# alenzhao/Mitty

Hardware: NVIDIA B200
Metric: read pairs/sec (2x150, FASTQ-formatted, corrupted) (higher is better)
Workload: dtype u8

## Files before the change

### mitty_b200/csrc/mg_core.cuh

```cuda
#pragma once
#include <stdint.h>

#if defined(__CUDACC__)
#define MG_HD __host__ __device__ __forceinline__
#else
#define MG_HD inline
#endif
#if defined(__CUDACC__)
#define MG_NI static __host__ __device__ __noinline__ __attribute__((unused))
#else
#define MG_NI static __attribute__((noinline, unused))
#endif
#if defined(__CUDA_ARCH__)
#define MG_UNROLL _Pragma("unroll")
#define MG_NOUNROLL _Pragma("unroll 1")
#else
#define MG_UNROLL
#define MG_NOUNROLL
#endif


struct alignas(16) MgNode {
  uint32_t key;
  int32_t pr;
// ... 1 lines not shown
  uint32_t op;
};

#define MG_EXC_CASE 1u
struct alignas(16) MgExc {
  uint32_t start;
  uint32_t len;
  uint32_t byte;
  uint32_t pad;
};


MG_HD uint32_t mg_funnel_r(uint32_t lo, uint32_t hi, uint32_t sh) {
#if defined(__CUDA_ARCH__)
  return __funnelshift_r(lo, hi, sh);
#else
  return sh ? ((lo >> sh) | (hi << (32 - sh))) : lo;
#endif
}

MG_HD uint32_t mg_funnel_l(uint32_t lo, uint32_t hi, uint32_t sh) {
#if defined(__CUDA_ARCH__)
  return __funnelshift_l(lo, hi, sh);
#else
  return sh ? ((hi << sh) | (lo >> (32 - sh))) : hi;
#endif
}

MG_HD uint32_t mg_brev(uint32_t x) {
#if defined(__CUDA_ARCH__)
  return __brev(x);
#else
  x = ((x >> 1) & 0x55555555u) | ((x & 0x55555555u) << 1);
  x = ((x >> 2) & 0x33333333u) | ((x & 0x33333333u) << 2);
  x = ((x >> 4) & 0x0F0F0F0Fu) | ((x & 0x0F0F0F0Fu) << 4);
  x = ((x >> 8) & 0x00FF00FFu) | ((x & 0x00FF00FFu) << 8);
  return (x >> 16) | (x << 16);
#endif
}

MG_HD uint32_t mg_prmt(uint32_t a, uint32_t sel) {
#if defined(__CUDA_ARCH__)
  return __byte_perm(a, 0u, sel);
#else
  uint32_t r = 0;
  for (int i = 0; i < 4; i++) r |= ((a >> (8 * ((sel >> (4 * i)) & 3))) & 0xFFu) << (8 * i);
  return r;
#endif
}

MG_HD uint32_t mg_prmt2(uint32_t a, uint32_t b, uint32_t sel) {
#if defined(__CUDA_ARCH__)
  return __byte_perm(a, b, sel);
#else
  const uint64_t ab = ((uint64_t)b << 32) | a;
  uint32_t r = 0;
  for (int i = 0; i < 4; i++) r |= (uint32_t)((ab >> (8 * ((sel >> (4 * i)) & 7))) & 0xFFu) << (8 * i);
  return r;
#endif
}

template <class P>
MG_HD uint32_t mg_codes16(P seq, int64_t s) {
  int64_t w = s >> 4;
  uint32_t sh = (uint32_t)(s & 15) * 2u;
  uint32_t lo = seq[w];
  uint32_t hi = sh ? seq[w + 1] : 0u;
  return mg_funnel_r(lo, hi, sh);
}

MG_HD uint32_t mg_revcomp16(uint32_t x) {
  uint32_t y = mg_brev(x);
  y = ((y >> 1) & 0x55555555u) | ((y & 0x55555555u) << 1);
  return ~y;
}

MG_HD uint32_t mg_chars4(uint32_t b) {
  uint32_t y = (b | (b << 4)) & 0x0F0Fu;
  uint32_t z = (y | (y << 2)) & 0x3333u;
  return mg_prmt(0x54474341u , z);
}

MG_HD uint32_t mg_base_code(uint8_t c) {
  return c == 'A' ? 0u : c == 'C' ? 1u : c == 'G' ? 2u : c == 'T' ? 3u : 4u;
}


struct MgPhilox { uint32_t v[4]; };

MG_HD void mg_mulhilo(uint32_t a, uint32_t b, uint32_t &hi, uint32_t &lo) {
  uint64_t p = (uint64_t)a * (uint64_t)b;
  hi = (uint32_t)(p >> 32); lo = (uint32_t)p;
}

template <int ROUNDS>
MG_HD MgPhilox mg_philox_r(uint32_t c0, uint32_t c1, uint32_t c2, uint32_t c3, uint32_t k0, uint32_t k1) {
  MG_UNROLL
  for (int r = 0; r < ROUNDS; r++) {
    uint32_t h0, l0, h1, l1;
    mg_mulhilo(0xD2511F53u, c0, h0, l0);
    mg_mulhilo(0xCD9E8D57u, c2, h1, l1);
    uint32_t n0 = h1 ^ c1 ^ k0, n2 = h0 ^ c3 ^ k1;
    c0 = n0; c1 = l1; c2 = n2; c3 = l0;
    k0 += 0x9E3779B9u; k1 += 0xBB67AE85u;
  }
  MgPhilox o; o.v[0] = c0; o.v[1] = c1; o.v[2] = c2; o.v[3] = c3;
  return o;
}

MG_HD MgPhilox mg_philox(uint32_t c0, uint32_t c1, uint32_t c2, uint32_t c3, uint32_t k0, uint32_t k1) {
  return mg_philox_r<10>(c0, c1, c2, c3, k0, k1);
}

#define MG_CORRUPT_ROUNDS 7
MG_HD MgPhilox mg_philox_corrupt(uint32_t c0, uint32_t c1, uint32_t c2, uint32_t k0, uint32_t k1) {
  return mg_philox_r<MG_CORRUPT_ROUNDS>(c0, c1, c2, 0x636f7272u , k0, k1);
}

MG_HD double mg_u53(uint32_t a, uint32_t b) {
  return ((double)(a >> 5) * 67108864.0 + (double)(b >> 6)) / 9007199254740992.0;
}

#define MG_STREAM_GAP 0x67617073u
#define MG_STREAM_TLEN 0x746c656eu
#define MG_STREAM_CORRUPT 0x636f7272u

MG_HD uint32_t mg_feistel_round(uint32_t r, uint32_t k) {
  uint32_t x = r * 0x9E3779B1u + k;
  x ^= x >> 15; x *= 0x85EBCA77u; x ^= x >> 13; x *= 0xC2B2AE3Du; x ^= x >> 16;
  return x;
}

MG_HD uint32_t mg_perm_bits(uint32_t n) {
  uint32_t bits = 2;
  while (bits < 32 && (1ull << bits) < (unsigned long long)n) bits++;
  return bits;
}

MG_HD uint32_t mg_permute(uint32_t i, uint32_t n, uint32_t bits, uint32_t k0, uint32_t k1) {
  const uint32_t wa = bits >> 1, ma = (1u << wa) - 1u, mb = (bits - wa >= 32u) ? 0xFFFFFFFFu : (1u << (bits - wa)) - 1u;
  do {
    uint32_t a = i & ma, b = (i >> wa) & mb;
    MG_UNROLL
    for (int t = 0; t < 6; t += 2) {
      a ^= mg_feistel_round(b, k0 + (uint32_t)t) & ma;
      b ^= mg_feistel_round(a, k1 + (uint32_t)t + 1u) & mb;
    }
    i = (b << wa) | a;
  } while (i >= n);
  return i;
}


MG_HD uint32_t mg_pow10(int d) {
  switch (d) {
    case 0: return 1u; case 1: return 10u; case 2: return 100u; case 3: return 1000u; case 4: return 10000u;
    case 5: return 100000u; case 6: return 1000000u; case 7: return 10000000u; case 8: return 100000000u;
    default: return 1000000000u;
  }
}

MG_HD int mg_ndigits_ones(uint32_t v, uint32_t &ones) {
  int d = 1; uint32_t o = 1u;
  if (v >= 10u) { d++; o += 10u; }
  if (v >= 100u) { d++; o += 100u; }
  if (v >= 1000u) { d++; o += 1000u; }
  if (v >= 10000u) { d++; o += 10000u; }
  if (v >= 100000u) { d++; o += 100000u; }
  if (v >= 1000000u) { d++; o += 1000000u; }
  if (v >= 10000000u) { d++; o += 10000000u; }
  if (v >= 100000000u) { d++; o += 100000000u; }
  if (v >= 1000000000u) { d++; o += 1000000000u; }
  ones = o;
  return d;
}

MG_HD int mg_ndigits32(uint32_t v) { uint32_t o; return mg_ndigits_ones(v, o); }

MG_HD int mg_ndigits(uint64_t v) {
  if (v <= 0xFFFFFFFFull) return mg_ndigits32((uint32_t)v);
  int d = 1;
  while (v >= 10) { v /= 10; d++; }
  return d;
}


MG_HD uint64_t mg_digit_sum(uint64_t m) {
  if (m == 0) return 0;
  if (m <= 0xFFFFFFFFull) {
    uint32_t ones;
    const int d = mg_ndigits_ones((uint32_t)m, ones);
    return (uint64_t)d * (m + 1) - (uint64_t)ones;
  }
  const int d = mg_ndigits(m);
  uint64_t ones = 0, p = 1;
  for (int k = 0; k < d; k++) { ones += p; p *= 10; }
  return (uint64_t)d * (m + 1) - ones;
}


struct MgCountWriter {
  static constexpr bool is_bytes = false;
  uint32_t n;
  MG_HD void put(uint8_t) { n++; }
  MG_HD void put_word(uint32_t) { n += 4; }
};

struct MgGenericSpace {
  static constexpr bool is_generic = true;
  typedef uint8_t *ptr;
  static MG_HD void st8(ptr p, uint8_t v) { *p = v; }
  static MG_HD void st32(ptr p, uint32_t v) { *reinterpret_cast<uint32_t *>(p) = v; }
  static MG_HD uint32_t ld32(ptr p) { return *reinterpret_cast<const uint32_t *>(p); }
  static MG_HD uint32_t ld8(ptr p) { return *p; }
  static MG_HD uint32_t low2(ptr p) { return (uint32_t)((uintptr_t)p & 3); }
};
#if defined(__CUDACC__)
struct MgSharedSpace {
  static constexpr bool is_generic = false;
  typedef uint32_t ptr;
  static __device__ __forceinline__ void st8(ptr p, uint8_t v) { asm volatile("st.shared.u8 [%0], %1;" ::"r"(p), "r"((uint32_t)v)); }
  static __device__ __forceinline__ void st32(ptr p, uint32_t v) { asm volatile("st.shared.b32 [%0], %1;" ::"r"(p), "r"(v)); }
  static __device__ __forceinline__ uint32_t ld32(ptr p) {
    uint32_t v;
    asm volatile("ld.shared.b32 %0, [%1];" : "=r"(v) : "r"(p));
    return v;
  }
  static __device__ __forceinline__ uint32_t ld8(ptr p) {
    uint32_t v;
    asm volatile("ld.shared.u8 %0, [%1];" : "=r"(v) : "r"(p));
    return v;
  }
  static __device__ __forceinline__ uint32_t low2(ptr p) { return p & 3u; }
};
#endif

template <class SP> MG_HD void mg_store_tail(typename SP::ptr b, uint32_t carry, uint32_t nb) {
  if (nb > 0) SP::st8(b, (uint8_t)carry);
  if (nb > 1) SP::st8(b + 1, (uint8_t)(carry >> 8));
  if (nb > 2) SP::st8(b + 2, (uint8_t)(carry >> 16));
}

struct MgTok { uint32_t lo, hi, n; };

template <class SP>
struct MgStream {
  static constexpr bool is_bytes = false;
  typename SP::ptr wp;
  uint32_t prev;
  uint32_t sh;
  uint32_t skip;

  MG_HD void begin(typename SP::ptr dst) {
    const uint32_t a = SP::low2(dst);
    wp = dst - a; sh = 8 * a; prev = 0u; skip = a;
  }
  MG_HD void begin_rmw(typename SP::ptr dst) {
    const uint32_t a = SP::low2(dst);
    wp = dst - a; sh = 8 * a; skip = 0;
    prev = a ? (SP::ld32(wp) << (32 - sh)) : 0u;
  }
  MG_HD void flush_word(uint32_t w) {
    if constexpr (SP::is_generic) {
      if (skip) { for (uint32_t i = skip; i < 4; i++) SP::st8(wp + i, (uint8_t)(w >> (8 * i))); skip = 0; wp += 4; return; }
    }
    SP::st32(wp, w); wp += 4;
  }
  MG_HD void put(uint8_t c) {
    prev = (prev >> 8) | ((uint32_t)c << 24);
    sh += 8;
    if (sh == 32) { flush_word(prev); sh = 0; }
  }
  MG_HD void put_word(uint32_t w) {
    flush_word(mg_funnel_l(prev, w, sh));
    prev = w;
  }
  MG_HD void append(MgTok t) {
    const uint32_t pend = mg_funnel_l(prev, 0u, sh);
    const uint32_t w0 = pend | (t.lo << sh);
    const uint32_t w1 = mg_funnel_l(t.lo, t.hi, sh);
    const uint32_t w2 = mg_funnel_l(t.hi, 0u, sh);
    const uint32_t tb = sh + 8u * t.n;
    if constexpr (SP::is_generic) {
      if (tb >= 32u) flush_word(w0);
      if (tb >= 64u) flush_word(w1);
    } else {
      if (tb >= 32u) SP::st32(wp, w0);
      if (tb >= 64u) SP::st32(wp + 4, w1);
      wp += (tb >> 3) & ~3u;
    }
    const uint32_t keep = tb >= 64u ? w2 : (tb >= 32u ? w1 : w0);
    sh = tb & 31u;
    prev = keep << ((32u - sh) & 31u);
  }
  MG_HD void end() {
    if (sh) {
      const uint32_t nb = sh >> 3, carry = prev >> (32 - sh);
      if constexpr (SP::is_generic) { const uint32_t k = skip; skip = 0; for (uint32_t i = k; i < nb; i++) SP::st8(wp + i, (uint8_t)(carry >> (8 * i))); }
      else mg_store_tail<SP>(wp, carry, nb);
    }
    sh = 0;
  }
  MG_HD void flush_own() { if (sh) flush_word(prev >> (32 - sh)); sh = 0; }
};


MG_HD uint32_t mg_dec4(uint32_t x) {
  const uint32_t c = (x * 5243u) >> 19;
  const uint32_t d = x - c * 100u;
  const uint32_t p = c | (d << 16);
  const uint32_t t = ((p * 103u) >> 10) & 0x000F000Fu;
  const uint32_t o = p - t * 10u;
  return (t | (o << 8)) + 0x30303030u;
}

MG_HD void mg_tok_num(uint32_t v, uint32_t pre, uint32_t npre, MgTok &A, MgTok &B) {
  const uint32_t top = v / 100000000u, low = v - top * 100000000u;
  const uint32_t a = low / 10000u, b = low - a * 10000u;
  uint32_t lo = mg_dec4(a), hi = mg_dec4(b);
  const uint32_t xl = lo ^ 0x30303030u, xh = hi ^ 0x30303030u;
  uint32_t lz;
#if defined(__CUDA_ARCH__)
  lz = xl ? ((uint32_t)__ffs((int)xl) - 1u) >> 3 : (xh ? 4u + (((uint32_t)__ffs((int)xh) - 1u) >> 3) : 7u);
#else
  lz = xl ? ((uint32_t)__builtin_ctz(xl)) >> 3 : (xh ? 4u + (((uint32_t)__builtin_ctz(xh)) >> 3) : 7u);
#endif
  if (top) lz = 0u;
  const bool big = lz >= 4u;
  const uint32_t l1 = big ? hi : lo, h1 = big ? 0u : hi, s2 = 8u * (lz & 3u);
  B.lo = mg_funnel_r(l1, h1, s2); B.hi = h1 >> s2; B.n = 8u - lz;
  const uint32_t tt = (top * 103u) >> 10, to = top - tt * 10u;
  const uint32_t nt = top >= 10u ? 2u : (top ? 1u : 0u);
  const uint32_t dig = top >= 10u ? ((tt + 48u) | ((to + 48u) << 8)) : (top ? to + 48u : 0u);
  const uint32_t ps = 8u * npre;
  A.lo = pre | (dig << ps); A.hi = mg_funnel_l(dig, 0u, ps); A.n = npre + nt;
}

template <class SP>
MG_HD void mg_put_num(MgStream<SP> &w, uint32_t v, uint32_t pre, uint32_t npre) {
  MgTok A, B;
  mg_tok_num(v, pre, npre, A, B);
  w.append(A); w.append(B);
}

template <class SP>
MG_HD void mg_put_small(MgStream<SP> &w, uint32_t v, uint32_t pre, uint32_t npre) {
  if (v >= 10000u) { mg_put_num(w, v, pre, npre); return; }
  const uint32_t d = mg_dec4(v), x = d ^ 0x30303030u;
  uint32_t lz;
#if defined(__CUDA_ARCH__)
  lz = (x & 0x00FFFFFFu) ? ((uint32_t)__ffs((int)x) - 1u) >> 3 : 3u;
#else
  lz = (x & 0x00FFFFFFu) ? ((uint32_t)__builtin_ctz(x)) >> 3 : 3u;
#endif
  const uint32_t dig = d >> (8u * lz), ps = 8u * npre;
  MgTok t;
  t.lo = pre | (dig << ps); t.hi = mg_funnel_l(dig, 0u, ps); t.n = npre + 4u - lz;
  w.append(t);
}

MG_HD MgTok mg_tok(uint32_t lo, uint32_t hi, uint32_t n) { MgTok t; t.lo = lo; t.hi = hi; t.n = n; return t; }

template <class W>
MG_HD void mg_put_u32(W &w, uint32_t v) {
  uint64_t acc = 0;
  int n = 0;
  do { uint32_t q = v / 10u; acc = (acc << 4) | (v - q * 10u); v = q; n++; } while (v);
  for (; n; n--) { w.put((uint8_t)('0' + ((uint32_t)acc & 15u))); acc >>= 4; }
}


template <class NP, class BP>
MG_NI int mg_find_node(NP nodes, BP blk, int blk_shift, int n_blk, int n_nodes, uint32_t x) {
  uint32_t b = x >> blk_shift;
  if ((int)b >= n_blk) b = (uint32_t)(n_blk - 1);
  int lo = (int)blk[b];
  int hi = ((int)b + 1 < n_blk) ? (int)blk[b + 1] : n_nodes - 1;
  while (lo < hi) {
    int mid = (lo + hi + 1) >> 1;
    if (nodes[mid].key <= x) lo = mid; else hi = mid - 1;
  }
  return lo;
}

template <class NP>
MG_HD int mg_last_node(NP nodes, int n0, int n_nodes, uint32_t x, int L) {
  const uint32_t last = x + (uint32_t)L - 1u;
  int n1 = n0;
  while (n1 + 1 < n_nodes && nodes[n1 + 1].key <= last) n1++;
  return n1;
}

MG_HD int32_t mg_read_pos(const MgNode &f, bool single, uint32_t x) {
  if (f.op == 'I') return single ? f.pr - 1 : f.pr;
  const int64_t ps0 = (int64_t)f.key - (f.op == 'D' ? 1 : 0);
  return (int32_t)((int64_t)x - ps0 + (int64_t)f.pr);
}

MG_HD int32_t mg_cigar_len(const MgNode &n, uint32_t x, int L) {
  if (n.op == 'D') return n.oplen;
  int64_t a = (int64_t)x - (int64_t)n.key; if (a < 0) a = 0;
  int64_t b = (int64_t)x + L - (int64_t)n.key; if ((int64_t)n.oplen < b) b = n.oplen;
  return (int32_t)(b - a);
}

template <class W>
MG_HD void mg_put_i32(W &w, int32_t v) {
  if (v < 0) { w.put('-'); mg_put_u32(w, (uint32_t)(-(int64_t)v)); } else mg_put_u32(w, (uint32_t)v);
}

MG_HD int mg_nchars_i32(int32_t v) { return v < 0 ? 1 + mg_ndigits32((uint32_t)(-(int64_t)v)) : mg_ndigits32((uint32_t)v); }

template <class NP>
MG_NI uint32_t mg_read_fields_len(NP nodes, int n0, int n1, uint32_t x, int L, int L_nd) {
  const MgNode f = nodes[n0];
  const bool single = (n0 == n1);
  uint32_t n = 2u + 1u + (uint32_t)mg_nchars_i32(mg_read_pos(f, single, x)) + 1u + (uint32_t)L_nd + 1u + 1u;
  if (single && f.op == '=') return n + (uint32_t)L_nd + 1u;
  if (single && f.op == 'I')
    return n + 1u + (uint32_t)mg_nchars_i32((int32_t)((int64_t)x - (int64_t)f.key)) + 1u + (uint32_t)L_nd + 1u + (uint32_t)mg_nchars_i32(f.oplen);
  uint32_t nv = 0;
  for (int k = n0; k <= n1; k++) {
    const MgNode nd = nodes[k];
    n += (uint32_t)mg_nchars_i32(mg_cigar_len(nd, x, L)) + 1u;
    if (nd.op != '=') {
      n += (nv ? 1u : 0u) + (nd.op == 'X' ? 1u : nd.op == 'I' ? (uint32_t)mg_nchars_i32(nd.oplen) : (uint32_t)mg_nchars_i32(-nd.oplen));
      nv++;
    }
  }
  return n;
}

template <class W, class NP>
MG_HD void mg_fmt_read(W &w, NP nodes, int n0, int n1, uint32_t x, int L, int strand) {
  const MgNode f = nodes[n0];
  const bool single = (n0 == n1);
  w.put('|'); w.put((uint8_t)('0' + strand));
  w.put('|'); mg_put_i32(w, mg_read_pos(f, single, x));
  w.put('|'); mg_put_u32(w, (uint32_t)L);
  w.put('|');
  if (single && f.op == '=') {
    mg_put_u32(w, (uint32_t)L); w.put('='); w.put('|');
    return;
  }
  if (single && f.op == 'I') {
    w.put('>'); mg_put_i32(w, (int32_t)((int64_t)x - (int64_t)f.key)); w.put(':'); mg_put_u32(w, (uint32_t)L); w.put('I');
  } else {
    for (int k = n0; k <= n1; k++) {
      const MgNode n = nodes[k];
      mg_put_i32(w, mg_cigar_len(n, x, L)); w.put((uint8_t)n.op);
    }
  }
  w.put('|');
  bool first = true;
  for (int k = n0; k <= n1; k++) {
    const MgNode n = nodes[k];
    if (n.op == '=') continue;
    if (!first) w.put(',');
    first = false;
    if (n.op == 'X') w.put('0');
    else mg_put_i32(w, n.op == 'I' ? n.oplen : -n.oplen);
  }
}

struct MgReadRef { uint32_t x; int n0, n1, strand; };

template <class W, class NP>
MG_HD void mg_fmt_qname(W &w, const uint8_t *prefix, int prefix_len, uint64_t cnt, bool with_cnt,
                        const uint8_t *mid, int mid_len, NP nodes, MgReadRef first, MgReadRef second, int L) {
  for (int i = 0; i < prefix_len; i++) w.put(prefix[i]);
  if (with_cnt) mg_put_u32(w, (uint32_t)cnt);
  for (int i = 0; i < mid_len; i++) w.put(mid[i]);
  MG_NOUNROLL
  for (int r = 0; r < 2; r++) {
    const MgReadRef R = r ? second : first;
    mg_fmt_read(w, nodes, R.n0, R.n1, R.x, L, R.strand);
  }
}

#define MG_QN_TOKS 24
struct MgQnConst {
  MgTok pre[MG_QN_TOKS], mid[MG_QN_TOKS];
  int n_pre, n_mid;
  MgTok tail[2], rl;
  uint32_t Lnd;
};

MG_HD MgTok mg_tok_bytes(const uint8_t *t, int from, int cnt) {
  MgTok k; k.lo = 0; k.hi = 0; k.n = (uint32_t)(cnt < 0 ? 0 : (cnt > 8 ? 8 : cnt));
  for (uint32_t i = 0; i < k.n; i++) { if (i < 4) k.lo |= (uint32_t)t[from + i] << (8 * i); else k.hi |= (uint32_t)t[from + i] << (8 * (i - 4)); }
  return k;
}

MG_HD void mg_qn_const(MgQnConst &Q, const uint8_t *prefix, int prefix_len, const uint8_t *mid, int mid_len, int L) {
  Q.n_pre = (prefix_len + 7) / 8; Q.n_mid = (mid_len + 7) / 8;
  for (int i = 0; i < Q.n_pre; i++) Q.pre[i] = mg_tok_bytes(prefix, 8 * i, prefix_len - 8 * i);
  for (int i = 0; i < Q.n_mid; i++) Q.mid[i] = mg_tok_bytes(mid, 8 * i, mid_len - 8 * i);
  uint8_t d[12], t[28]; int nd = 0, n = 0;
  uint32_t v = (uint32_t)L;
  do { d[nd++] = (uint8_t)('0' + v % 10u); v /= 10u; } while (v);
  t[n++] = '|';
  for (int i = nd - 1; i >= 0; i--) t[n++] = d[i];
  t[n++] = '|';
  const int nrl = n;
  for (int i = nd - 1; i >= 0; i--) t[n++] = d[i];
  t[n++] = '='; t[n++] = '|';
  const bool ok = n <= 16;
  Q.Lnd = ok ? (uint32_t)nd : 0u;
  Q.rl = mg_tok_bytes(t, 0, ok ? nrl : 0);
  Q.tail[0] = mg_tok_bytes(t, 0, ok ? n : 0);
  Q.tail[1] = mg_tok_bytes(t, 8, ok ? n - 8 : 0);
}

template <class SP, class NP>
MG_HD void mg_put_read(MgStream<SP> &w, const MgQnConst &Q, NP nodes, MgReadRef R, int L) {
  const MgNode f = nodes[R.n0];
  const bool single = (R.n0 == R.n1);
  mg_put_num(w, (uint32_t)mg_read_pos(f, single, R.x), (uint32_t)'|' | ((uint32_t)('0' + R.strand) << 8) | ((uint32_t)'|' << 16), 3u);
  if (single && f.op == '=' && Q.Lnd) {
    w.append(Q.tail[0]); w.append(Q.tail[1]);
    return;
  }
  if (Q.Lnd) w.append(Q.rl); else mg_put_num(w, (uint32_t)L, '|', 1u), w.append(mg_tok('|', 0, 1));
  if (single && f.op == '=') {
    mg_put_num(w, (uint32_t)L, 0u, 0u); w.append(mg_tok((uint32_t)'=' | ((uint32_t)'|' << 8), 0, 2));
    return;
  }
  if (single && f.op == 'I') {
    mg_put_small(w, (uint32_t)((int64_t)R.x - (int64_t)f.key), '>', 1u);
    mg_put_small(w, (uint32_t)L, ':', 1u);
    mg_put_small(w, (uint32_t)f.oplen, (uint32_t)'I' | ((uint32_t)'|' << 8), 2u);
    return;
  }
  const int k1 = R.n0 + 1 <= R.n1 ? R.n0 + 1 : R.n1, k2 = R.n0 + 2 <= R.n1 ? R.n0 + 2 : R.n1;
  const MgNode c1 = nodes[k1], c2 = nodes[k2];
  auto node_at = [&](int k) -> MgNode { const int d = k - R.n0; if (d == 0) return f; if (d == 1) return c1; if (d == 2) return c2; return nodes[k]; };
  uint32_t pre = 0, npre = 0;
  for (int k = R.n0; k <= R.n1; k++) {
    const MgNode n = node_at(k);
    mg_put_small(w, (uint32_t)mg_cigar_len(n, R.x, L), pre, npre);
    pre = n.op; npre = 1;
  }
  pre |= (uint32_t)'|' << 8; npre = 2;
  bool firstv = true;
  for (int k = R.n0; k <= R.n1; k++) {
    const MgNode n = node_at(k);
    if (n.op == '=') continue;
    if (!firstv) { pre = ','; npre = 1; }
    firstv = false;
    if (n.op == 'D') { pre |= (uint32_t)'-' << (8 * npre); npre++; }
    mg_put_small(w, n.op == 'X' ? 0u : (uint32_t)n.oplen, pre, npre);
    npre = 0; pre = 0;
  }
  if (npre) w.append(mg_tok(pre, 0, npre));
}

template <class SP, class NP, class STR>
MG_HD void mg_put_qname(MgStream<SP> &w, const MgQnConst &Q, const STR &str, uint32_t cnt, NP nodes, MgReadRef first, MgReadRef second, int L) {
  for (int i = 0; i < str.n_pre; i++) w.append(str.pre[i]);
  mg_put_num(w, cnt, 0u, 0u);
  for (int i = 0; i < str.n_mid; i++) w.append(str.mid[i]);
  MG_NOUNROLL
  for (int r = 0; r < 2; r++) mg_put_read(w, Q, nodes, r ? second : first, L);
  w.append(mg_tok('\n', 0, 1));
// ... 472 lines not shown
```

### mitty_b200/csrc/mg_kernels.cu

```cuda
#include <algorithm>
#include <cstdlib>
#include "mg_internal.h"

#define FULL 0xffffffffu


__device__ __forceinline__ uint32_t warp_incl_scan_u32(uint32_t v, int lane) {
#pragma unroll
  for (int d = 1; d < 32; d <<= 1) {
    uint32_t n = __shfl_up_sync(FULL, v, d);
    if (lane >= d) v += n;
  }
  return v;
}

__device__ __forceinline__ unsigned long long warp_sum_u64(unsigned long long v) {
#pragma unroll
  for (int d = 16; d >= 1; d >>= 1) v += __shfl_xor_sync(FULL, v, d);
  return v;
}

__device__ __forceinline__ unsigned long long ld_vol64(const unsigned long long *p) {
  return *(const volatile unsigned long long *)p;
}
// ... 388 lines not shown
#pragma unroll
  for (int q = 0; q < 4; q++) {
    uint32_t i = i0 + 2 * q;
    MgPhilox r = mg_philox(i >> 1, 0u, 0u, MG_STREAM_GAP, k0, k1);
#pragma unroll
    for (int h = 0; h < 2; h++) {
      double u = mg_u53(r.v[2 * h], r.v[2 * h + 1]);
      double gd = ceil(log(1.0 - u) * inv_log1mp);
      uint32_t gv = gd < 1.0 ? 1u : (gd > 4.0e9 ? 4000000000u : (uint32_t)gd);
      g[2 * q + h] = (i + h < n) ? gv : 0u;
    }
  }
}

__global__ void __launch_bounds__(GAP_THREADS) k_gap_partial(uint32_t n, double inv_log1mp, uint32_t k0, uint32_t k1,
                                                             unsigned long long *partial) {
  __shared__ unsigned long long s_w[GAP_THREADS / 32];
  uint32_t i0 = blockIdx.x * GAP_PER_BLOCK + threadIdx.x * GAP_PER_THREAD;
  uint32_t g[8];
  unsigned long long sum = 0;
  if (i0 < n) { gaps8(i0, n, inv_log1mp, k0, k1, g); for (int q = 0; q < 8; q++) sum += g[q]; }
  sum = warp_sum_u64(sum);
  if ((threadIdx.x & 31) == 0) s_w[threadIdx.x >> 5] = sum;
  __syncthreads();
  if (threadIdx.x == 0) {
    unsigned long long t = 0;
    for (int w = 0; w < GAP_THREADS / 32; w++) t += s_w[w];
    partial[blockIdx.x] = t;
  }
}

__global__ void __launch_bounds__(1024) k_scan_partials_u64(unsigned long long *partial, int n) {
  __shared__ unsigned long long s_w[32];
  __shared__ unsigned long long s_carry;
  int lane = threadIdx.x & 31, wid = threadIdx.x >> 5;
  if (threadIdx.x == 0) s_carry = 0;
  __syncthreads();
  for (int base = 0; base < n; base += 1024) {
    int i = base + threadIdx.x;
    unsigned long long v = (i < n) ? partial[i] : 0, x = v;
#pragma unroll
    for (int d = 1; d < 32; d <<= 1) { unsigned long long y = __shfl_up_sync(FULL, x, d); if (lane >= d) x += y; }
    if (lane == 31) s_w[wid] = x;
    __syncthreads();
    if (wid == 0) {
      unsigned long long t = s_w[lane], xx = t;
#pragma unroll
      for (int d = 1; d < 32; d <<= 1) { unsigned long long y = __shfl_up_sync(FULL, xx, d); if (lane >= d) xx += y; }
      s_w[lane] = xx - t;
    }
    __syncthreads();
    unsigned long long carry = s_carry;
    unsigned long long incl = carry + s_w[wid] + x;
    if (i < n) partial[i] = incl - v;
    __syncthreads();
    if (threadIdx.x == 1023) s_carry = incl;
    __syncthreads();
  }
}

__global__ void __launch_bounds__(GAP_THREADS) k_gap_final(uint32_t n, double inv_log1mp, uint32_t k0, uint32_t k1,
                                                           const unsigned long long *__restrict__ partial, uint32_t *__restrict__ ts_sorted) {
  __shared__ unsigned long long s_w[GAP_THREADS / 32];
  uint32_t i0 = blockIdx.x * GAP_PER_BLOCK + threadIdx.x * GAP_PER_THREAD;
  int lane = threadIdx.x & 31, wid = threadIdx.x >> 5;
  uint32_t g[8];
  unsigned long long sum = 0;
  if (i0 < n) { gaps8(i0, n, inv_log1mp, k0, k1, g); for (int q = 0; q < 8; q++) sum += g[q]; }
  else { for (int q = 0; q < 8; q++) g[q] = 0; }
  unsigned long long x = sum;
#pragma unroll
  for (int d = 1; d < 32; d <<= 1) { unsigned long long y = __shfl_up_sync(FULL, x, d); if (lane >= d) x += y; }
  if (lane == 31) s_w[wid] = x;
  __syncthreads();
  unsigned long long off = partial[blockIdx.x];
  for (int w = 0; w < wid; w++) off += s_w[w];
  unsigned long long run = off + x - sum;
  if (i0 < n) {
#pragma unroll
    for (int q = 0; q < 8; q++) {
      run += g[q];
      if (i0 + q < n) {
        unsigned long long v = run + 1;
        ts_sorted[i0 + q] = v > 0xFFFFFFFFull ? 0xFFFFFFFFu : (uint32_t)v;
      }
    }
  }
}

void mg_launch_gap_scan(uint32_t n, double p, uint32_t k0, uint32_t k1, uint32_t *ts_sorted, unsigned long long *partial,
                        cudaStream_t st) {
  if (n == 0) return;
  double inv = 1.0 / log(1.0 - p);
  int nb = (int)((n + GAP_PER_BLOCK - 1) / GAP_PER_BLOCK);
  k_gap_partial<<<nb, GAP_THREADS, 0, st>>>(n, inv, k0, k1, partial);
  k_scan_partials_u64<<<1, 1024, 0, st>>>(partial, nb);
  k_gap_final<<<nb, GAP_THREADS, 0, st>>>(n, inv, k0, k1, partial, ts_sorted);
}


struct Cand { int64_t ts_rel; int64_t te_rel; uint32_t fo; bool k1; };

__device__ __forceinline__ Cand sample_candidate(const MgUnitParams &P, const uint32_t *s_alias, uint32_t j) {
  Cand c;
  int64_t tl;
  c.fo = 0;
  if (P.mode == MG_MODE_PHILOX) {
    uint32_t i = mg_permute(j, P.n_cand, P.perm_bits, P.key_perm0, P.key_perm1);
    c.ts_rel = (int64_t)P.ts_sorted[i];
    MgPhilox r = mg_philox(j, 0u, 0u, MG_STREAM_TLEN, P.key_tlen0, P.key_tlen1);
    if (P.tlen_alias) {
      const uint32_t idx = r.v[0] >> 22, e = s_alias[idx];
      tl = (r.v[0] & 0x3FFFFFu) < (e >> 10) ? idx : (e & 1023u);
    } else {
      tl = mg_lower_bound_f64(P.cum_tlen, P.n_tlen, mg_u53(r.v[0], r.v[1]));
    }
    c.fo = r.v[2] & 1u;
  } else {
    c.ts_rel = P.ts_in[j] - P.p_min;
    tl = (P.mode == MG_MODE_DET) ? (int64_t)mg_lower_bound_f64(P.cum_tlen, P.n_tlen, P.u_tlen[j]) : P.tl_in[j];
  }
  if (tl < P.rlen) tl = P.rlen;
  c.te_rel = c.ts_rel + tl;
  c.k1 = (c.te_rel < (int64_t)P.hap_len) && (c.ts_rel >= 0);
  return c;
}

__global__ void __launch_bounds__(256) k_sample(MgSampleParams S) {
  __shared__ uint32_t s_tlen[MG_TLEN_K];
  if (S.u.mode == MG_MODE_PHILOX && S.u.tlen_alias)
    for (int i = threadIdx.x; i < MG_TLEN_K; i += blockDim.x) s_tlen[i] = S.u.tlen_alias[i];
  __syncthreads();
  for (uint32_t j = blockIdx.x * blockDim.x + threadIdx.x; j < S.u.n_cand; j += gridDim.x * blockDim.x) {
    Cand c = sample_candidate(S.u, s_tlen, j);
    S.ts_out[j] = c.ts_rel + S.u.p_min;
    S.te_out[j] = c.k1 ? c.te_rel + S.u.p_min : -1;
    S.fo_out[j] = (int8_t)c.fo;
  }
}

void mg_launch_sample(const MgSampleParams &P, cudaStream_t st) {
  if (P.u.n_cand == 0) return;
  int grid = (int)((P.u.n_cand + 255) / 256);
  if (grid > 148 * 8) grid = 148 * 8;
  k_sample<<<grid, 256, 0, st>>>(P);
}


struct Agg { unsigned long long c1, c2, by; };

#define DESC_FLAG(x) ((uint32_t)((x) >> 62))
#define DESC_MASK62 ((1ull << 62) - 1ull)

__device__ Agg tile_lookback(const MgUnitParams &P, int tile, int lane) {
  Agg ex = {0, 0, 0};
  int idx = tile - 1;
  while (true) {
    int t = idx - lane;
    unsigned long long a = 0, b = 0;
    uint32_t fl = 2;
    if (t >= 0) {
      do {
        a = ld_vol64(P.descA + t);
        b = ld_vol64(P.descB + t);
      } while (DESC_FLAG(a) == 0 || DESC_FLAG(a) != DESC_FLAG(b));
      fl = DESC_FLAG(a);
    }
    __syncwarp();
    uint32_t pm = __ballot_sync(FULL, fl == 2);
    int first = __ffs(pm) - 1;
    bool take = (t >= 0) && (first < 0 || lane <= first);
    unsigned long long c1 = take ? ((a >> 31) & 0x7FFFFFFFull) : 0;
    unsigned long long c2 = take ? (a & 0x7FFFFFFFull) : 0;
    unsigned long long by = take ? (b & DESC_MASK62) : 0;
    ex.c1 += warp_sum_u64(c1); ex.c2 += warp_sum_u64(c2); ex.by += warp_sum_u64(by);
    if (first >= 0) break;
    idx -= 32;
  }
  return ex;
}

#define PLAN_THREADS 256

__global__ void __launch_bounds__(PLAN_THREADS) k_unit_plan(const __grid_constant__ MgUnitParams P) {
  __shared__ uint32_t s_tlen[MG_TLEN_K];
  __shared__ uint32_t s_wc[PLAN_THREADS / 32], s_ws[PLAN_THREADS / 32];
  __shared__ unsigned long long s_base[3];
  __shared__ uint32_t s_tile;
  const int t = threadIdx.x, lane = t & 31, wid = t >> 5;
  const int L = P.rlen;
  if (P.mode == MG_MODE_PHILOX && P.tlen_alias) {
#pragma unroll 1
    for (int i = t; i < MG_TLEN_K; i += PLAN_THREADS) s_tlen[i] = P.tlen_alias[i];
  }
  while (true) {
    __syncthreads();
    if (t == 0) s_tile = atomicAdd(P.tile_counter, 1u);
    __syncthreads();
    const int tile = (int)s_tile;
    if (tile >= P.n_tiles) break;
    const uint32_t j = (uint32_t)tile * PLAN_THREADS + t;
    bool k1 = false, k2 = false, ta = false, tb = false;
    uint32_t xa = 0, xb = 0, fo = 0, sz = 0;
    int n0a = 0, n1a = 0, n0b = 0, n1b = 0;
    if (j < P.n_cand) {
      Cand c = sample_candidate(P, s_tlen, j);
      k1 = c.k1; fo = c.fo;
      if (k1) {
        xa = (uint32_t)c.ts_rel; xb = (uint32_t)(c.te_rel - L);
        k2 = true;
        if (P.n_exc) {
          const MgExcView ev = {P.exc, P.eblk, P.blk_shift, P.n_blk};
          const int na = mg_count_N(ev, P.n_exc, xa, L, ta), nb = mg_count_N(ev, P.n_exc, xb, L, tb);
          k2 = na <= 2 && nb <= 2;
        }
        if (k2) {
          n0a = mg_find_node(P.nodes, P.blk, P.blk_shift, P.n_blk, P.n_nodes, xa);
          n1a = mg_last_node(P.nodes, n0a, P.n_nodes, xa, L);
          n0b = mg_find_node(P.nodes, P.blk, P.blk_shift, P.n_blk, P.n_nodes, xb);
          n1b = mg_last_node(P.nodes, n0b, P.n_nodes, xb, L);
          sz = (uint32_t)P.qn_len + mg_read_fields_len(P.nodes, n0a, n1a, xa, L, P.L_nd) +
               mg_read_fields_len(P.nodes, n0b, n1b, xb, L, P.L_nd) + 2u * (uint32_t)L + 5u;
        }
      }
    }
    const uint32_t cpk = (k1 ? 1u : 0u) | (k2 ? 0x10000u : 0u);
    const uint32_t ic = warp_incl_scan_u32(cpk, lane), is = warp_incl_scan_u32(sz, lane);
    if (lane == 31) { s_wc[wid] = ic; s_ws[wid] = is; }
    __syncthreads();
    uint32_t oc = 0, os = 0, tc = 0, ts_ = 0;
#pragma unroll
    for (int w = 0; w < PLAN_THREADS / 32; w++) {
      if (w < wid) { oc += s_wc[w]; os += s_ws[w]; }
      tc += s_wc[w]; ts_ += s_ws[w];
    }
    const uint32_t ec = oc + ic - cpk, es = os + is - sz;
    const uint32_t tile_c1 = tc & 0xFFFFu, tile_c2 = tc >> 16, tile_sz = ts_;
    if (wid == 0) {
      Agg ex = {0, 0, 0};
      if (tile > 0) {
        if (lane == 0) {
          st_vol64(P.descA + tile, (1ull << 62) | ((unsigned long long)tile_c1 << 31) | tile_c2);
          st_vol64(P.descB + tile, (1ull << 62) | tile_sz);
        }
        ex = tile_lookback(P, tile, lane);
      }
      if (lane == 0) {
        const unsigned long long i1 = ex.c1 + tile_c1, i2 = ex.c2 + tile_c2, ib = ex.by + tile_sz;
        st_vol64(P.descA + tile, (2ull << 62) | (i1 << 31) | i2);
        st_vol64(P.descB + tile, (2ull << 62) | ib);
        s_base[0] = ex.c1; s_base[1] = ex.c2; s_base[2] = ex.by;
        if (tile == P.n_tiles - 1) { P.totals[0] = i1; P.totals[1] = i2; P.totals[2] = ib + mg_digit_sum(i2); }
      }
    }
    __syncthreads();
    if (k2) {
      const unsigned long long base1 = s_base[0], base2 = s_base[1];
      const unsigned long long rank = base2 + (ec >> 16);
      const unsigned long long off = s_base[2] + es + mg_digit_sum(rank);
      const uint32_t my_fo = (P.mode == MG_MODE_PHILOX) ? fo : (uint32_t)(P.fo_in[base1 + (ec & 0xFFFFu)] & 1);
      MgPlan pl;
      pl.xa = xa; pl.xb = xb; pl.n0a = n0a; pl.n0b = n0b;
      pl.dn = (uint32_t)(n1a - n0a) | ((uint32_t)(n1b - n0b) << 16);
      pl.fo_sz = (my_fo << 31) | ((ta ? 1u : 0u) << 30) | ((tb ? 1u : 0u) << 29) | (sz + (uint32_t)mg_ndigits32((uint32_t)(rank + 1)));
      pl.off = off;
      P.plan[rank] = pl;
    }
  }
}

void mg_launch_plan(const MgUnitParams &P, cudaStream_t st) {
  if (P.n_tiles == 0) return;
  int grid = P.n_tiles < 148 * 8 ? P.n_tiles : 148 * 8;
  k_unit_plan<<<grid, PLAN_THREADS, 0, st>>>(P);
}

__global__ void __launch_bounds__(PLAN_THREADS) k_batch_plan(const __grid_constant__ MgUnitParams P) {
  __shared__ uint32_t s_ts[MG_BATCH_MAXC];
  __shared__ uint32_t s_tlen[MG_TLEN_K];
  __shared__ unsigned long long s_w64[PLAN_THREADS / 32];
  __shared__ uint32_t s_wc[PLAN_THREADS / 32], s_ws[PLAN_THREADS / 32];
  __shared__ unsigned long long s_carry[3];
  const int t = threadIdx.x, lane = t & 31, wid = t >> 5;
  const int L = P.rlen;
  const MgBatchUnit U = P.bunits[blockIdx.x];
  const uint32_t n = U.n_cand;
  const MgUnitKeys K = mg_unit_keys(U.seed, n);
  if (P.mode == MG_MODE_PHILOX) {
    if (P.tlen_alias) for (int i = t; i < MG_TLEN_K; i += PLAN_THREADS) s_tlen[i] = P.tlen_alias[i];
    uint32_t g[8];
    unsigned long long sum = 0;
    const uint32_t i0 = (uint32_t)t * 8u;
    if (i0 < n) { gaps8(i0, n, P.inv_log1mp, K.gap0, K.gap1, g); for (int q = 0; q < 8; q++) sum += g[q]; }
    else { for (int q = 0; q < 8; q++) g[q] = 0; }
    unsigned long long x = sum;
#pragma unroll
    for (int d = 1; d < 32; d <<= 1) { unsigned long long y = __shfl_up_sync(FULL, x, d); if (lane >= d) x += y; }
    if (lane == 31) s_w64[wid] = x;
    __syncthreads();
    unsigned long long run = x - sum;
    for (int w = 0; w < wid; w++) run += s_w64[w];
    for (int q = 0; q < 8; q++) {
      run += g[q];
      if (i0 + q < n) { const unsigned long long v = run + 1; s_ts[i0 + q] = v > 0xFFFFFFFFull ? 0xFFFFFFFFu : (uint32_t)v; }
    }
  }
  if (t == 0) { s_carry[0] = 0; s_carry[1] = 0; s_carry[2] = 0; }
  __syncthreads();
  for (uint32_t c0 = 0; c0 < n; c0 += PLAN_THREADS) {
    const uint32_t j = c0 + t;
    bool k1 = false, k2 = false, ta = false, tb = false;
    uint32_t xa = 0, xb = 0, fo = 0, sz = 0;
    int n0a = 0, n1a = 0, n0b = 0, n1b = 0;
    if (j < n) {
      int64_t ts_rel, tl;
      if (P.mode == MG_MODE_PHILOX) {
        const uint32_t i = mg_permute(j, n, K.perm_bits, K.perm0, K.perm1);
        ts_rel = (int64_t)s_ts[i];
        const MgPhilox r = mg_philox(j, 0u, 0u, MG_STREAM_TLEN, K.tlen0, K.tlen1);
        if (P.tlen_alias) { const uint32_t idx = r.v[0] >> 22, e = s_tlen[idx]; tl = (r.v[0] & 0x3FFFFFu) < (e >> 10) ? idx : (e & 1023u); }
        else tl = mg_lower_bound_f64(P.cum_tlen, P.n_tlen, mg_u53(r.v[0], r.v[1]));
        fo = r.v[2] & 1u;
      } else {
        ts_rel = P.ts_in[U.draw_off + j] - U.p_min;
        tl = mg_lower_bound_f64(P.cum_tlen, P.n_tlen, P.u_tlen[U.draw_off + j]);
      }
      if (tl < L) tl = L;
      const int64_t te_rel = ts_rel + tl;
      k1 = te_rel < (int64_t)U.hap_len && ts_rel >= 0;
      if (k1) {
        xa = U.x0 + (uint32_t)ts_rel; xb = U.x0 + (uint32_t)(te_rel - L);
        k2 = true;
        if (P.n_exc) {
          const MgExcView ev = {P.exc, P.eblk, P.blk_shift, P.n_blk};
          const int na = mg_count_N(ev, P.n_exc, xa, L, ta), nb = mg_count_N(ev, P.n_exc, xb, L, tb);
          k2 = na <= 2 && nb <= 2;
        }
        if (k2) {
          n0a = mg_find_node(P.nodes, P.blk, P.blk_shift, P.n_blk, P.n_nodes, xa);
          n1a = mg_last_node(P.nodes, n0a, P.n_nodes, xa, L);
          n0b = mg_find_node(P.nodes, P.blk, P.blk_shift, P.n_blk, P.n_nodes, xb);
          n1b = mg_last_node(P.nodes, n0b, P.n_nodes, xb, L);
          sz = U.qn_len + mg_read_fields_len(P.nodes, n0a, n1a, xa, L, P.L_nd) + mg_read_fields_len(P.nodes, n0b, n1b, xb, L, P.L_nd) + 2u * (uint32_t)L + 5u;
        }
      }
    }
    const uint32_t cpk = (k1 ? 1u : 0u) | (k2 ? 0x10000u : 0u);
    const uint32_t ic = warp_incl_scan_u32(cpk, lane), is = warp_incl_scan_u32(sz, lane);
    if (lane == 31) { s_wc[wid] = ic; s_ws[wid] = is; }
    __syncthreads();
    uint32_t oc = 0, os = 0, tc = 0, ts_ = 0;
#pragma unroll
    for (int w = 0; w < PLAN_THREADS / 32; w++) {
      if (w < wid) { oc += s_wc[w]; os += s_ws[w]; }
      tc += s_wc[w]; ts_ += s_ws[w];
    }
    const uint32_t ec = oc + ic - cpk, es = os + is - sz;
    const unsigned long long base1 = s_carry[0], base2 = s_carry[1], baseb = s_carry[2];
    if (k2) {
      const unsigned long long rank = base2 + (ec >> 16);
      const unsigned long long off = baseb + es + mg_digit_sum(rank);
      const uint32_t my_fo = (P.mode == MG_MODE_PHILOX) ? fo : (uint32_t)(P.fo_in[U.draw_off + base1 + (ec & 0xFFFFu)] & 1);
      MgPlan pl;
      pl.xa = xa; pl.xb = xb; pl.n0a = n0a; pl.n0b = n0b;
      pl.dn = (uint32_t)(n1a - n0a) | ((uint32_t)(n1b - n0b) << 16);
      pl.fo_sz = (my_fo << 31) | ((ta ? 1u : 0u) << 30) | ((tb ? 1u : 0u) << 29) | (sz + (uint32_t)mg_ndigits32((uint32_t)(rank + 1)));
      pl.off = off | ((unsigned long long)blockIdx.x << 40);
      P.plan[U.plan_off + rank] = pl;
    }
    __syncthreads();
    if (t == 0) { s_carry[0] = base1 + (tc & 0xFFFFu); s_carry[1] = base2 + (tc >> 16); s_carry[2] = baseb + ts_; }
    __syncthreads();
  }
  if (t == 0) {
    P.unit_te[blockIdx.x] = (long long)s_carry[0];
    P.unit_kept[blockIdx.x] = (long long)s_carry[1];
    P.unit_bytes[blockIdx.x] = (long long)(s_carry[2] + mg_digit_sum(s_carry[1]));
  }
}

void mg_launch_batch_plan(const MgUnitParams &P, cudaStream_t st) {
  if (P.n_bunits == 0) return;
  k_batch_plan<<<P.n_bunits, PLAN_THREADS, 0, st>>>(P);
}


template <int CORRUPT, class STR>
__device__ __noinline__ void emit_oversize(uint8_t *dst, uint32_t qlen, const MgUnitParams &P, const STR &str, const MgCorruptCtx &cor,
                                           unsigned long long cnt, MgReadRef first, MgReadRef second, MgReadRef mine, int f) {
  const int L = P.rlen;
  MgSeqSrc<0, const uint32_t *> S;
  S.load(P.hap, mine.x, L, mine.strand);
  if constexpr (CORRUPT) {
    mg_emit_frame_qname<MgGenericSpace>(dst, P.qn, str, (uint32_t)cnt, P.nodes, first, second, L);
    mg_emit_frame_seps<MgGenericSpace>(dst, qlen, L);
    mg_emit_seq_corrupt<MgGenericSpace, CORRUPT == 2>(dst + qlen + 1, dst + qlen + 1 + L + 3, S, MgExcView{P.exc, P.eblk, P.blk_shift, P.n_blk}, P.n_exc, cor, (uint32_t)(cnt - 1), (uint32_t)f, (uint32_t)f);
  } else {
    MgStream<MgGenericSpace> ws;
    mg_emit_record<MgGenericSpace>(ws, dst, P.qn, str, (uint32_t)cnt, P.nodes, first, second, S);
    ws.end();
    if (P.n_exc) mg_patch_exc<MgGenericSpace>(dst + (qlen + 1), MgExcView{P.exc, P.eblk, P.blk_shift, P.n_blk}, P.n_exc, S.hap, S.x, L, S.strand);
  }
}

__device__ __forceinline__ void bulk_store(uint8_t *gdst, uint32_t ssrc, uint32_t bytes, unsigned long long policy) {
  asm volatile("cp.async.bulk.global.shared::cta.bulk_group.L2::cache_hint [%0], [%1], %2, %3;"
               :: "l"(gdst), "r"(ssrc), "r"(bytes), "l"(policy) : "memory");
  asm volatile("cp.async.bulk.commit_group;" ::: "memory");
}

template <int MAXW, int CORRUPT, bool BATCH = false>
__global__ void __launch_bounds__(MG_CTA, 4) k_unit_emit(const __grid_constant__ MgUnitParams P) {
  extern __shared__ __align__(16) uint8_t smem[];
  const int t = threadIdx.x, lane = t & 31, wid = t >> 5;
  uint8_t *stage = smem + (uint32_t)wid * (uint32_t)(P.stage_cap + 16);
  uint32_t stage_s = (uint32_t)__cvta_generic_to_shared(stage);
  asm volatile("" : "+r"(stage_s));
  const int L = P.rlen;
  const MgExcView ev = {P.exc, P.eblk, P.blk_shift, P.n_blk};
  const unsigned long long n_kept = BATCH ? (unsigned long long)P.kept_base[P.n_bunits] : P.totals[1];
  const unsigned long long n_bytes = BATCH ? (unsigned long long)P.byte_base[P.n_bunits] : P.totals[2];
  if (n_bytes > P.cap) { if (t == 0 && blockIdx.x == 0) P.totals[3] = 1ull; return; }
  if (n_kept == 0) return;
  unsigned long long policy = 0;
  if (P.bulk) asm volatile("createpolicy.fractional.L2::evict_first.b64 %0, 1.0;" : "=l"(policy));
  bool in_flight = false;
  const unsigned long long n_wt = (n_kept + 31) / 32;
// ... 602 lines not shown
```

Baseline: 1.366 billion.

## Software-pipeline plan kernel lookback, widen lookback window, branchless digit counting

```diff
diff --git a/mitty_b200/csrc/mg_core.cuh b/mitty_b200/csrc/mg_core.cuh
--- a/mitty_b200/csrc/mg_core.cuh
+++ b/mitty_b200/csrc/mg_core.cuh
@@ -177,27 +177,25 @@
 }
 
 
-MG_HD uint32_t mg_pow10(int d) {
-  switch (d) {
-    case 0: return 1u; case 1: return 10u; case 2: return 100u; case 3: return 1000u; case 4: return 10000u;
-    case 5: return 100000u; case 6: return 1000000u; case 7: return 10000000u; case 8: return 100000000u;
-    default: return 1000000000u;
-  }
+MG_HD uint32_t mg_pow10(uint32_t d) {
+  return ((d & 1u) ? 10u : 1u) * ((d & 2u) ? 100u : 1u) * ((d & 4u) ? 10000u : 1u) * ((d & 8u) ? 100000000u : 1u);
+}
+
+MG_HD uint32_t mg_bit_length(uint32_t v) {
+#if defined(__CUDA_ARCH__)
+  return 32u - (uint32_t)__clz((int)v);
+#else
+  return 32u - (uint32_t)__builtin_clz(v);
+#endif
 }
 
 MG_HD int mg_ndigits_ones(uint32_t v, uint32_t &ones) {
-  int d = 1; uint32_t o = 1u;
-  if (v >= 10u) { d++; o += 10u; }
-  if (v >= 100u) { d++; o += 100u; }
-  if (v >= 1000u) { d++; o += 1000u; }
-  if (v >= 10000u) { d++; o += 10000u; }
-  if (v >= 100000u) { d++; o += 100000u; }
-  if (v >= 1000000u) { d++; o += 1000000u; }
-  if (v >= 10000000u) { d++; o += 10000000u; }
-  if (v >= 100000000u) { d++; o += 100000000u; }
-  if (v >= 1000000000u) { d++; o += 1000000000u; }
-  ones = o;
-  return d;
+  const uint32_t w = v | 1u;
+  const uint32_t t = (mg_bit_length(w) * 1233u) >> 12;
+  const uint32_t p = mg_pow10(t);
+  const bool up = w >= p;
+  ones = (p - 1u) / 9u + (up ? p : 0u);
+  return (int)(t + (up ? 1u : 0u));
 }
 
 MG_HD int mg_ndigits32(uint32_t v) { uint32_t o; return mg_ndigits_ones(v, o); }
@@ -434,7 +432,10 @@
   if (v < 0) { w.put('-'); mg_put_u32(w, (uint32_t)(-(int64_t)v)); } else mg_put_u32(w, (uint32_t)v);
 }
 
-MG_HD int mg_nchars_i32(int32_t v) { return v < 0 ? 1 + mg_ndigits32((uint32_t)(-(int64_t)v)) : mg_ndigits32((uint32_t)v); }
+MG_HD int mg_nchars_i32(int32_t v) {
+  const bool neg = v < 0;
+  return (neg ? 1 : 0) + mg_ndigits32(neg ? (uint32_t)(-(int64_t)v) : (uint32_t)v);
+}
 
 template <class NP>
 MG_NI uint32_t mg_read_fields_len(NP nodes, int n0, int n1, uint32_t x, int L, int L_nd) {
diff --git a/mitty_b200/csrc/mg_kernels.cu b/mitty_b200/csrc/mg_kernels.cu
--- a/mitty_b200/csrc/mg_kernels.cu
+++ b/mitty_b200/csrc/mg_kernels.cu
@@ -564,58 +564,76 @@
 #define DESC_FLAG(x) ((uint32_t)((x) >> 62))
 #define DESC_MASK62 ((1ull << 62) - 1ull)
 
+#define LOOKBACK_WIN 128
 __device__ Agg tile_lookback(const MgUnitParams &P, int tile, int lane) {
+  constexpr int Q = LOOKBACK_WIN / 32;
   Agg ex = {0, 0, 0};
   int idx = tile - 1;
   while (true) {
-    int t = idx - lane;
-    unsigned long long a = 0, b = 0;
-    uint32_t fl = 2;
-    if (t >= 0) {
-      do {
-        a = ld_vol64(P.descA + t);
-        b = ld_vol64(P.descB + t);
-      } while (DESC_FLAG(a) == 0 || DESC_FLAG(a) != DESC_FLAG(b));
-      fl = DESC_FLAG(a);
+    unsigned long long a[Q], b[Q];
+#pragma unroll
+    for (int q = 0; q < Q; q++) {
+      const int t = idx - 32 * q - lane;
+      a[q] = 2ull << 62; b[q] = 2ull << 62;
+      if (t >= 0) { a[q] = ld_vol64(P.descA + t); b[q] = ld_vol64(P.descB + t); }
+    }
+#pragma unroll
+    for (int q = 0; q < Q; q++) {
+      const int t = idx - 32 * q - lane;
+      while (t >= 0 && (DESC_FLAG(a[q]) == 0 || DESC_FLAG(a[q]) != DESC_FLAG(b[q]))) {
+        a[q] = ld_vol64(P.descA + t); b[q] = ld_vol64(P.descB + t);
+      }
     }
     __syncwarp();
-    uint32_t pm = __ballot_sync(FULL, fl == 2);
-    int first = __ffs(pm) - 1;
-    bool take = (t >= 0) && (first < 0 || lane <= first);
-    unsigned long long c1 = take ? ((a >> 31) & 0x7FFFFFFFull) : 0;
-    unsigned long long c2 = take ? (a & 0x7FFFFFFFull) : 0;
-    unsigned long long by = take ? (b & DESC_MASK62) : 0;
+    int stop = LOOKBACK_WIN;
+#pragma unroll
+    for (int q = Q - 1; q >= 0; q--) {
+      const uint32_t pm = __ballot_sync(FULL, DESC_FLAG(a[q]) == 2);
+      if (pm) stop = 32 * q + __ffs(pm) - 1;
+    }
+    unsigned long long c1 = 0, c2 = 0, by = 0;
+#pragma unroll
+    for (int q = 0; q < Q; q++) {
+      if (32 * q + lane <= stop) {
+        c1 += (a[q] >> 31) & 0x7FFFFFFFull; c2 += a[q] & 0x7FFFFFFFull; by += b[q] & DESC_MASK62;
+      }
+    }
     ex.c1 += warp_sum_u64(c1); ex.c2 += warp_sum_u64(c2); ex.by += warp_sum_u64(by);
-    if (first >= 0) break;
-    idx -= 32;
+    if (stop < LOOKBACK_WIN) break;
+    idx -= LOOKBACK_WIN;
   }
   return ex;
 }
 
 #define PLAN_THREADS 256
 
-__global__ void __launch_bounds__(PLAN_THREADS) k_unit_plan(const __grid_constant__ MgUnitParams P) {
+__global__ void __launch_bounds__(PLAN_THREADS, 6) k_unit_plan(const __grid_constant__ MgUnitParams P) {
   __shared__ uint32_t s_tlen[MG_TLEN_K];
-  __shared__ uint32_t s_wc[PLAN_THREADS / 32], s_ws[PLAN_THREADS / 32];
-  __shared__ unsigned long long s_base[3];
-  __shared__ uint32_t s_tile;
+  __shared__ uint4 s_hold[2][PLAN_THREADS];
+  __shared__ uint2 s_hold2[2][PLAN_THREADS], s_ex[PLAN_THREADS];
+  __shared__ uint32_t s_wc[2][PLAN_THREADS / 32], s_ws[2][PLAN_THREADS / 32];
+  __shared__ unsigned long long s_base[2][3];
+  __shared__ uint32_t s_tile[2];
   const int t = threadIdx.x, lane = t & 31, wid = t >> 5;
   const int L = P.rlen;
   if (P.mode == MG_MODE_PHILOX && P.tlen_alias) {
 #pragma unroll 1
     for (int i = t; i < MG_TLEN_K; i += PLAN_THREADS) s_tlen[i] = P.tlen_alias[i];
   }
-  while (true) {
-    __syncthreads();
-    if (t == 0) s_tile = atomicAdd(P.tile_counter, 1u);
-    __syncthreads();
-    const int tile = (int)s_tile;
-    if (tile >= P.n_tiles) break;
+  if (t == 0) s_tile[0] = atomicAdd(P.tile_counter, 1u);
+  __syncthreads();
+  int tile = (int)s_tile[0], prev = -1;
+  uint32_t prev_c1 = 0, prev_c2 = 0, prev_sz = 0;
+#pragma unroll 1
+  for (int k = 0;; k++) {
+    const int cur = k & 1;
+    const bool live = tile < P.n_tiles;
+    if (t == 0 && live) s_tile[cur ^ 1] = atomicAdd(P.tile_counter, 1u);
     const uint32_t j = (uint32_t)tile * PLAN_THREADS + t;
     bool k1 = false, k2 = false, ta = false, tb = false;
     uint32_t xa = 0, xb = 0, fo = 0, sz = 0;
     int n0a = 0, n1a = 0, n0b = 0, n1b = 0;
-    if (j < P.n_cand) {
+    if (live && j < P.n_cand) {
       Cand c = sample_candidate(P, s_tlen, j);
       k1 = c.k1; fo = c.fo;
       if (k1) {
@@ -636,55 +654,73 @@
         }
       }
     }
+    s_hold[cur][t] = make_uint4(xa, xb, (uint32_t)n0a, (uint32_t)n0b);
+    s_hold2[cur][t] = make_uint2((uint32_t)(n1a - n0a) | ((uint32_t)(n1b - n0b) << 16),
+                                 (fo << 31) | ((ta ? 1u : 0u) << 30) | ((tb ? 1u : 0u) << 29) | sz);
     const uint32_t cpk = (k1 ? 1u : 0u) | (k2 ? 0x10000u : 0u);
     const uint32_t ic = warp_incl_scan_u32(cpk, lane), is = warp_incl_scan_u32(sz, lane);
-    if (lane == 31) { s_wc[wid] = ic; s_ws[wid] = is; }
+    if (lane == 31) { s_wc[cur][wid] = ic; s_ws[cur][wid] = is; }
+    if (wid == 0 && prev >= 0) {
+      Agg ex = {0, 0, 0};
+      if (prev > 0) ex = tile_lookback(P, prev, lane);
+      if (lane == 0) {
+        const unsigned long long i1 = ex.c1 + prev_c1, i2 = ex.c2 + prev_c2, ib = ex.by + prev_sz;
+        if (prev > 0) {
+          st_vol64(P.descA + prev, (2ull << 62) | (i1 << 31) | i2);
+          st_vol64(P.descB + prev, (2ull << 62) | ib);
+        }
+        s_base[cur ^ 1][0] = ex.c1; s_base[cur ^ 1][1] = ex.c2; s_base[cur ^ 1][2] = ex.by;
+        if (prev == P.n_tiles - 1) { P.totals[0] = i1; P.totals[1] = i2; P.totals[2] = ib + mg_digit_sum(i2); }
+      }
+    }
     __syncthreads();
+    if (prev >= 0) {
+      const uint2 h1 = s_hold2[cur ^ 1][t];
+      if (h1.y & 0x1FFFFFFFu) {
+        const uint4 h0 = s_hold[cur ^ 1][t];
+        const uint2 ex = s_ex[t];
+        const unsigned long long base1 = s_base[cur ^ 1][0], base2 = s_base[cur ^ 1][1];
+        const unsigned long long rank = base2 + (ex.x >> 16);
+        const unsigned long long off = s_base[cur ^ 1][2] + ex.y + mg_digit_sum(rank);
+        const uint32_t my_fo = (P.mode == MG_MODE_PHILOX) ? h1.y >> 31 : (uint32_t)(P.fo_in[base1 + (ex.x & 0xFFFFu)] & 1);
+        MgPlan pl;
+        pl.xa = h0.x; pl.xb = h0.y; pl.n0a = (int32_t)h0.z; pl.n0b = (int32_t)h0.w;
+        pl.dn = h1.x;
+        pl.fo_sz = (my_fo << 31) | ((h1.y & 0x7FFFFFFFu) + (uint32_t)mg_ndigits32((uint32_t)(rank + 1)));
+        pl.off = off;
+        P.plan[rank] = pl;
+      }
+    }
+    if (!live) break;
     uint32_t oc = 0, os = 0, tc = 0, ts_ = 0;
 #pragma unroll
     for (int w = 0; w < PLAN_THREADS / 32; w++) {
-      if (w < wid) { oc += s_wc[w]; os += s_ws[w]; }
-      tc += s_wc[w]; ts_ += s_ws[w];
+      if (w < wid) { oc += s_wc[cur][w]; os += s_ws[cur][w]; }
+      tc += s_wc[cur][w]; ts_ += s_ws[cur][w];
     }
     const uint32_t ec = oc + ic - cpk, es = os + is - sz;
-    const uint32_t tile_c1 = tc & 0xFFFFu, tile_c2 = tc >> 16, tile_sz = ts_;
-    if (wid == 0) {
-      Agg ex = {0, 0, 0};
-      if (tile > 0) {
-        if (lane == 0) {
-          st_vol64(P.descA + tile, (1ull << 62) | ((unsigned long long)tile_c1 << 31) | tile_c2);
-          st_vol64(P.descB + tile, (1ull << 62) | tile_sz);
-        }
-        ex = tile_lookback(P, tile, lane);
-      }
-      if (lane == 0) {
-        const unsigned long long i1 = ex.c1 + tile_c1, i2 = ex.c2 + tile_c2, ib = ex.by + tile_sz;
-        st_vol64(P.descA + tile, (2ull << 62) | (i1 << 31) | i2);
-        st_vol64(P.descB + tile, (2ull << 62) | ib);
-        s_base[0] = ex.c1; s_base[1] = ex.c2; s_base[2] = ex.by;
-        if (tile == P.n_tiles - 1) { P.totals[0] = i1; P.totals[1] = i2; P.totals[2] = ib + mg_digit_sum(i2); }
-      }
-    }
-    __syncthreads();
-    if (k2) {
-      const unsigned long long base1 = s_base[0], base2 = s_base[1];
-      const unsigned long long rank = base2 + (ec >> 16);
-      const unsigned long long off = s_base[2] + es + mg_digit_sum(rank);
-      const uint32_t my_fo = (P.mode == MG_MODE_PHILOX) ? fo : (uint32_t)(P.fo_in[base1 + (ec & 0xFFFFu)] & 1);
-      MgPlan pl;
-      pl.xa = xa; pl.xb = xb; pl.n0a = n0a; pl.n0b = n0b;
-      pl.dn = (uint32_t)(n1a - n0a) | ((uint32_t)(n1b - n0b) << 16);
-      pl.fo_sz = (my_fo << 31) | ((ta ? 1u : 0u) << 30) | ((tb ? 1u : 0u) << 29) | (sz + (uint32_t)mg_ndigits32((uint32_t)(rank + 1)));
-      pl.off = off;
-      P.plan[rank] = pl;
-    }
+    prev_c1 = tc & 0xFFFFu; prev_c2 = tc >> 16; prev_sz = ts_;
+    if (t == 0) {
+      const unsigned long long fl = tile == 0 ? 2ull << 62 : 1ull << 62;
+      st_vol64(P.descA + tile, fl | ((unsigned long long)prev_c1 << 31) | prev_c2);
+      st_vol64(P.descB + tile, fl | prev_sz);
+    }
+    s_ex[t] = make_uint2(ec, es);
+    prev = tile;
+    tile = (int)s_tile[cur ^ 1];
   }
 }
 
 void mg_launch_plan(const MgUnitParams &P, cudaStream_t st) {
   if (P.n_tiles == 0) return;
-  int grid = P.n_tiles < 148 * 8 ? P.n_tiles : 148 * 8;
-  k_unit_plan<<<grid, PLAN_THREADS, 0, st>>>(P);
+  static const int resident = [] {
+    int dev = 0, sms = 0, per_sm = 0;
+    cudaGetDevice(&dev);
+    cudaDeviceGetAttribute(&sms, cudaDevAttrMultiProcessorCount, dev);
+    cudaOccupancyMaxActiveBlocksPerMultiprocessor(&per_sm, k_unit_plan, PLAN_THREADS, 0);
+    return std::max(1, sms * per_sm);
+  }();
+  k_unit_plan<<<std::min(P.n_tiles, resident), PLAN_THREADS, 0, st>>>(P);
 }
 
 __global__ void __launch_bounds__(PLAN_THREADS) k_batch_plan(const __grid_constant__ MgUnitParams P) {
```

After: 1.414 billion, median of 6. 1.04x the previous value.
